# acdha/trivy

Hardware: AMD Instinct MI355X
Metric: secret-scan GB/s (builtin rules) at 1/2/4/8 MI355X; % of HBM peak (higher is better)
Workload: dtype u8

## Files before the change

include/trivy_secret.h:

```cpp
#ifndef TRIVY_SECRET_H
#define TRIVY_SECRET_H

#include <stddef.h>
#include <stdint.h>

#ifdef __cplusplus
extern "C" {
#endif

#define TSG_OK 0
#define TSG_ERR_CONFIG -1
#define TSG_ERR_ARG -2
#define TSG_ERR_GPU -3
#define TSG_ERR_NOMEM -4
#define TSG_ERR_INTERNAL -5

typedef struct tsg_allow_rule_desc {
  const char* id;
  const char* description;
  const char* regex;
  const char* path;
} tsg_allow_rule_desc;

typedef struct tsg_rule_desc {
// ... 230 lines not shown
int tsg_emulate_candidates(const tsg_ruleset* rs, const uint8_t* data, const uint64_t* offsets,
                           uint32_t nfiles, uint32_t chunk, uint32_t ext_cap, uint64_t items_cap,
                           uint32_t max_dense, uint32_t word_recs, uint32_t* records,
                           size_t records_cap, uint64_t* n_records);

int tsg_emulate_item_candidates(const tsg_ruleset* rs, const uint8_t* data, const uint64_t* offsets,
                                uint32_t nfiles, uint32_t chunk, uint32_t ext_cap, uint32_t* triples,
                                size_t triples_cap, uint64_t* n_triples);

int tsg_expand_candidates(const tsg_ruleset* rs, const uint8_t* data, const uint64_t* offsets,
                          uint32_t nfiles, const uint32_t* records, size_t n_records,
                          uint32_t* triples, size_t triples_cap, uint64_t* n_triples);

int tsg_layout_reference(const uint64_t* counts, uint32_t n_groups, uint64_t nchunks,
                         uint64_t items_cap, uint32_t max_dense, uint8_t* kind, uint64_t* totals);

int tsg_emulate_k1(const tsg_ruleset* rs, const uint8_t* data, const uint64_t* offsets,
                   uint32_t nfiles, uint32_t chunk, uint32_t* kw, size_t kw_len, uint32_t* ev,
                   size_t ev_len);

int tsg_emulate_k1f(const tsg_ruleset* rs, const uint8_t* data, const uint64_t* offsets,
                    uint32_t nfiles, uint32_t chunk, const uint32_t* quiet_ids, uint32_t nquiet,
                    uint32_t sample_kib, uint32_t* kw, size_t kw_len, uint32_t* ev, size_t ev_len,
                    uint64_t* stats);

int tsg_ruleset_rule_plan(const tsg_ruleset* rs, uint32_t rule, int32_t* group, int32_t* relax,
                          int64_t* max_len);

int tsg_ruleset_rule_anchor(const tsg_ruleset* rs, uint32_t rule, uint32_t* event, int64_t* evdist,
                            char* desc, size_t desc_len);

int tsg_ruleset_k1_literal(const tsg_ruleset* rs, uint32_t i, uint8_t* buf, uint32_t cap,
                           uint32_t* len, uint32_t* event);

int tsg_scan_batch_emulated(const tsg_ruleset* rs, const uint8_t* data, const uint64_t* offsets,
                            uint32_t nfiles, const char* paths, const uint64_t* path_offsets,
                            uint32_t chunk, tsg_result** out);

typedef struct tsg_layer tsg_layer;
typedef struct tsg_layer_view {
  const uint8_t* data;
  const uint64_t* offsets;
  uint32_t nfiles;
  const uint8_t* paths;
  const uint64_t* path_offsets;
  const char* opq;
  size_t opq_len;
  const char* wh;
  size_t wh_len;
  uint32_t walked;
} tsg_layer_view;
int tsg_layer_pack(const tsg_ruleset* rs, const uint8_t* tar, uint64_t tar_len,
                   const char* const* skip_files, uint32_t n_skip_files,
                   const char* const* skip_dirs, uint32_t n_skip_dirs, const char* config_path,
                   tsg_layer** out);
int tsg_layer_pack_shard(const tsg_ruleset* rs, const uint8_t* tar, uint64_t tar_len,
                         const char* const* skip_files, uint32_t n_skip_files,
                         const char* const* skip_dirs, uint32_t n_skip_dirs, const char* config_path,
                         uint32_t rank, uint32_t world, tsg_layer** out);
int tsg_layer_get(const tsg_layer* layer, tsg_layer_view* out);
typedef struct tsg_layer_range tsg_layer_range;
int tsg_layer_range_walk(const uint8_t* tar, uint64_t tar_len, uint32_t rank, uint32_t world,
                         tsg_layer_range** out, uint64_t info[4]);
int tsg_layer_range_sync(tsg_layer_range* range, uint64_t pos, uint64_t* end);
int tsg_layer_range_dirs(tsg_layer_range* range, const char* const* skip_dirs, uint32_t n_skip_dirs,
                         const char** out, uint64_t* out_len);
// ... 65 lines not shown
```

trivy_amd/_native.py:

```python
import ctypes as C
import os

LIB_PATH = os.path.join(os.path.dirname(os.path.abspath(__file__)), "libtrivy_secret.so")
if os.environ.get("TSG_LIB_VARIANT"):
    LIB_PATH = os.path.join(os.path.dirname(os.path.abspath(__file__)),
                            "libtrivy_secret_%s.so" % os.environ["TSG_LIB_VARIANT"])

TSG_OK = 0
TSG_ERR_CONFIG = -1
TSG_ERR_ARG = -2
TSG_ERR_GPU = -3
TSG_ERR_NOMEM = -4
TSG_ERR_INTERNAL = -5


class AllowRuleDesc(C.Structure):
    _fields_ = [("id", C.c_char_p), ("description", C.c_char_p), ("regex", C.c_char_p),
                ("path", C.c_char_p)]


class RuleDesc(C.Structure):
    _fields_ = [("id", C.c_char_p), ("category", C.c_char_p), ("title", C.c_char_p),
                ("severity", C.c_char_p), ("regex", C.c_char_p),
                ("keywords", C.POINTER(C.c_char_p)), ("n_keywords", C.c_uint32),
# ... 200 lines not shown
                                       C.POINTER(C.c_char_p), C.c_uint32, C.POINTER(C.c_char_p),
                                       C.c_uint32, C.c_char_p, C.POINTER(_P)]),
    ("tsg_layer_range_free", None, [_P]),
    ("tsg_fs_pack", C.c_int, [_P, C.c_char_p, C.POINTER(C.c_char_p), C.c_uint32,
                              C.POINTER(C.c_char_p), C.c_uint32, C.c_char_p, C.POINTER(_P)]),
    ("tsg_fs_pack_shard", C.c_int, [_P, C.c_char_p, C.POINTER(C.c_char_p), C.c_uint32,
                                    C.POINTER(C.c_char_p), C.c_uint32, C.c_char_p, C.c_uint32,
                                    C.c_uint32, C.POINTER(_P)]),
    ("tsg_layer_pack_slot", C.c_int, [_P, _P, C.c_uint64, C.POINTER(C.c_char_p), C.c_uint32,
                                      C.POINTER(C.c_char_p), C.c_uint32, C.c_char_p,
                                      C.POINTER(C.c_uint32), C.POINTER(_P)]),
    ("tsg_layer_range_pack_slot", C.c_int, [_P, _P, C.POINTER(C.c_char_p), C.c_uint32,
                                            C.POINTER(C.c_char_p), C.c_uint32,
                                            C.POINTER(C.c_char_p), C.c_uint32, C.c_char_p,
                                            C.POINTER(C.c_uint32), C.POINTER(_P)]),
    ("tsg_fs_pack_slot", C.c_int, [_P, C.c_char_p, C.POINTER(C.c_char_p), C.c_uint32,
                                   C.POINTER(C.c_char_p), C.c_uint32, C.c_char_p,
                                   C.POINTER(C.c_uint32), C.POINTER(_P)]),
    ("tsg_layer_scan", C.c_int, [_P, _P, C.c_uint64, C.POINTER(C.c_char_p), C.c_uint32,
                                 C.POINTER(C.c_char_p), C.c_uint32, C.c_char_p, C.POINTER(_P),
                                 C.POINTER(_P)]),
    ("tsg_fs_scan", C.c_int, [_P, C.c_char_p, C.POINTER(C.c_char_p), C.c_uint32,
                              C.POINTER(C.c_char_p), C.c_uint32, C.c_char_p, C.POINTER(_P),
                              C.POINTER(_P)]),
    ("tsg_layer_free", None, [_P]),
    ("tsg_go_sort_perm", C.c_int, [_P, _U64P, _I64P, C.c_uint32, C.POINTER(C.c_uint32)]),
    ("tsg_ruleset_rule_anchor", C.c_int, [_P, C.c_uint32, C.POINTER(C.c_uint32),
                                          C.POINTER(C.c_int64), C.c_char_p, C.c_size_t]),
    ("tsg_emulate_k1f", C.c_int, [_P, _P, _U64P, C.c_uint32, C.c_uint32, C.POINTER(C.c_uint32),
                                  C.c_uint32, C.c_uint32, C.POINTER(C.c_uint32), C.c_size_t,
                                  C.POINTER(C.c_uint32), C.c_size_t, C.POINTER(C.c_uint64)]),
    ("tsg_ruleset_k1_literal", C.c_int, [_P, C.c_uint32, C.c_char_p, C.c_uint32,
                                         C.POINTER(C.c_uint32), C.POINTER(C.c_uint32)]),
]

_lib = None


def lib():
    global _lib
    if _lib is None:
        if not os.path.exists(LIB_PATH):
            raise ImportError("libtrivy_secret.so is not built; run `python -m trivy_amd.build` "
                              "(expected at %s)" % LIB_PATH)
        L = C.CDLL(LIB_PATH)
        for name, res, args in SIGNATURES:
            fn = getattr(L, name)
            fn.restype = res
            fn.argtypes = args
        _lib = L
    return _lib


class NativeError(RuntimeError):
    def __init__(self, code, msg):
        super().__init__("%s (code %d)" % (msg, code))
        self.code = code


def knob(name, value=None):
    check(lib().tsg_test_knob(name.encode(), None if value is None else str(value).encode()))


def check(rc):
    if rc != TSG_OK:
        raise NativeError(rc, lib().tsg_last_error().decode("utf-8", "replace"))
# ... 2 lines not shown
```

trivy_amd/csrc/capi.cpp:

```cpp
#include <chrono>
#include <cstdio>
#include <cstdlib>
#include <cstring>
#include <exception>
#include <thread>

#include "internal.hpp"
#include "k1f.hpp"

namespace tsg {

static thread_local std::string g_last_error;

void set_error(const std::string& msg) { g_last_error = msg; }
int fail(int code, const std::string& msg) {
  g_last_error = msg;
  return code;
}

static void copy_err(const std::string& m, char* err, size_t len) {
  if (!err || len == 0) return;
  size_t n = std::min(len - 1, m.size());
  std::memcpy(err, m.data(), n);
  err[n] = 0;
// ... 402 lines not shown
      stats[0] = st[0];
      stats[1] = st[1];
      stats[2] = t.nlit;
      stats[3] = 0;
    }
    return TSG_OK;
  } catch (const std::bad_alloc&) {
    return fail(TSG_ERR_NOMEM, "out of memory");
  } catch (const std::exception& ex) {
    return fail(TSG_ERR_INTERNAL, ex.what());
  }
}

int tsg_ruleset_rule_plan(const tsg_ruleset* rs, uint32_t rule, int32_t* group, int32_t* relax,
                          int64_t* max_len) {
  if (!rs || rule >= rs->rs.rules.size()) return fail(TSG_ERR_ARG, "bad argument");
  const Plan& p = *rs->plan;
  if (group) *group = p.rule_hostonly[rule] ? -1 : p.rule_group[rule];
  if (relax) *relax = p.rule_relax[rule];
  if (max_len) *max_len = p.rule_maxlen[rule];
  return TSG_OK;
}

int tsg_ruleset_rule_anchor(const tsg_ruleset* rs, uint32_t rule, uint32_t* event, int64_t* evdist,
                            char* desc, size_t desc_len) {
  if (!rs || rule >= rs->rs.rules.size()) return fail(TSG_ERR_ARG, "bad argument");
  const Plan& p = *rs->plan;
  if (event) *event = p.rule_event[rule];
  if (evdist) *evdist = p.rule_evdist[rule];
  copy_err(p.rule_anchor[rule], desc, desc_len);
  return TSG_OK;
}

int tsg_ruleset_k1_literal(const tsg_ruleset* rs, uint32_t i, uint8_t* buf, uint32_t cap,
                           uint32_t* len, uint32_t* event) {
  if (!rs || (!buf && cap)) return fail(TSG_ERR_ARG, "bad argument");
  const Plan& p = *rs->plan;
  if (i >= p.k1_lits.size()) return fail(TSG_ERR_ARG, "no such K1 literal");
  const std::string& s = p.k1_lits[i];
  if (buf) std::memcpy(buf, s.data(), std::min<size_t>(cap, s.size()));
  if (len) *len = (uint32_t)s.size();
  if (event) *event = p.lit_event[i];
  return TSG_OK;
}

int tsg_go_sort_perm(const uint8_t* keys, const uint64_t* key_offsets, const int64_t* secondary,
                     uint32_t n, uint32_t* perm) {
  if ((n && (!keys || !key_offsets || !perm))) return fail(TSG_ERR_ARG, "bad argument");
  try {
    go_sort_perm(keys, key_offsets, secondary, n, perm);
    return TSG_OK;
  } catch (const std::bad_alloc&) {
    return fail(TSG_ERR_NOMEM, "out of memory");
  }
}

const uint8_t* tsg_result_data(const tsg_result* r, size_t* len) {
  if (!r) {
    if (len) *len = 0;
    return nullptr;
  }
  if (len) *len = r->buf.size();
  return (const uint8_t*)r->buf.data();
}

void tsg_result_free(tsg_result* r) { delete r; }
// ... 101 lines not shown
```

trivy_amd/csrc/k1f.cpp:

```cpp
#include "k1f.hpp"

#include <algorithm>
#include <cmath>
#include <cstring>
#include <memory>

namespace tsg {

namespace {

const uint32_t kBigram[] = {
#include "bigram.inc"
};

uint8_t fold(uint8_t c) { return (c >= 'A' && c <= 'Z') ? (uint8_t)(c + 32) : c; }

struct TextModel {
  std::vector<double> pi;
  std::vector<double> trans;
  TextModel() : pi(256, 0), trans(256 * 256, 0) {
    std::vector<double> cnt(256 * 256, 0.01);
    for (uint32_t e : kBigram) cnt[(e & 0xFF) * 256 + ((e >> 8) & 0xFF)] += std::exp2((double)(e >> 16) / 16.0) - 1.0;
    double tot = 0;
    for (int a = 0; a < 256; a++) {
// ... 299 lines not shown
          const uint32_t m = L.len - o >= 4 ? 0xFFFFFFFFu : (1u << (8 * (L.len - o))) - 1;
          ok = ((k1f_lower4(load4((int64_t)(s + o))) & m) == lv);
        }
        if (!ok) continue;
        stats[1]++;
        (*ev)[e / chunk] |= L.ev;
        if (L.kw >= 0) {
          const uint32_t f = (uint32_t)(std::upper_bound(bv.offsets, bv.offsets + F + 1, e) - bv.offsets) - 1;
          if (s >= bv.offsets[f]) (*kw)[(size_t)f * W + L.kw / 32] |= 1u << (L.kw % 32);
        }
      }
    }
  };
  uint32_t m1 = 0, m2 = 0;
  for (uint64_t P = 0; P < total; P += 16) {
    uint32_t r[16];
    for (int k = 0; k < 16; k++) r[k] = R((int64_t)(P + k));
    uint32_t any = 0;
    for (int g = 0; g < 4; g++) {
      const uint32_t gr = r[4 * g] | r[4 * g + 1] | r[4 * g + 2] | r[4 * g + 3];
      if (!(gr & 0xFFFFu)) continue;
      stats[0]++;
      any |= gr;
      for (int k = 4 * g; k < 4 * g + 4; k++)
        if (P + k < total && (r[k] & 0xFFFFu)) verify(P + k, r[k] & 0xFFFFu);
    }
    (void)any;
    const uint32_t m = k1f_flags(r[3], r[7], r[11], r[15]);
    const uint32_t rb = k1f_runs(m, m1, m2);
    if (rb) (*ev)[P / chunk] |= rb;
    m2 = m1;
    m1 = m;
  }
}

}
```

trivy_amd/csrc/kernels.hip:

```cpp
#include <hip/hip_runtime.h>

#include <algorithm>
#include <map>
#include <cstdlib>
#include <cstring>
#include <memory>
#include <vector>

#include "device.hpp"
#include "internal.hpp"
#include "k1f.hpp"

namespace tsg {

#define HIP_TRY(x)                                                                    \
  do {                                                                                \
    hipError_t e_ = (x);                                                              \
    if (e_ != hipSuccess)                                                             \
      return fail(TSG_ERR_GPU, std::string(#x) + ": " + hipGetErrorString(e_));       \
  } while (0)

constexpr int kStreams = 4;
constexpr int kK1Chains = 2;
constexpr int kK1Unroll = 8;
// ... 1445 lines not shown
    __syncthreads();
  }
}

struct GateArgs {
  const uint32_t* ev;
  uint64_t nchunks;
  uint32_t* evlist;
  uint32_t* nev;
  uint32_t ev_blocks;
  const uint32_t* kw;
  uint32_t F, W, GW;
  const unsigned long long* kwg;
  const unsigned long long* galw;
  unsigned long long* ggate;
  unsigned long long* clk;
  uint32_t kwg_lds;
};
constexpr uint32_t kKwgLdsMax = 48 * 1024;
__global__ void __launch_bounds__(kBlock) gates_kernel(GateArgs A) {
  extern __shared__ __attribute__((aligned(16))) uint8_t smem[];
  if (threadIdx.x == 0 && blockIdx.x < kStampBlocks)
    atomicMax(&A.clk[kClkGatesStart], ~(unsigned long long)wall_clock64());
  if (blockIdx.x < A.ev_blocks) {
    ev_compact_block(A.ev, A.nchunks, A.evlist, A.nev, blockIdx.x, A.ev_blocks);
  } else {
    const unsigned long long* kwg = A.kwg;
    if (A.kwg_lds) {
      stage16(smem, A.kwg, A.kwg_lds);
      __syncthreads();
      kwg = (const unsigned long long*)smem;
    }
    ggate_file((blockIdx.x - A.ev_blocks) * blockDim.x + threadIdx.x, A.kw, A.F, A.W, kwg, A.galw, A.GW, A.ggate);
  }
}

static inline size_t item_lds_host(uint32_t G, uint32_t GW) { return 256 * (size_t)GW + 8 * (size_t)G; }
constexpr uint32_t kItemKwgLdsMax = 16 * 1024;
struct ItemLds {
  const unsigned long long* gofbit;
  const uint32_t* gback;
  const uint32_t* gevents;
  const unsigned long long* kwg;
};
__device__ __forceinline__ uint32_t item_lds_bytes(const ItemArgs& A) { return 256 * A.GW + 8 * A.G + A.kwg_lds; }
__device__ __forceinline__ ItemLds item_lds_load(const ItemArgs& A, uint8_t* smem) {
  unsigned long long* gofbit = (unsigned long long*)smem;
  uint32_t* gback = (uint32_t*)(gofbit + 32 * A.GW);
  uint32_t* gevents = gback + A.G;
  for (uint32_t i = threadIdx.x; i < 32 * A.GW; i += blockDim.x) gofbit[i] = A.gofbit[i];
  for (uint32_t i = threadIdx.x; i < A.G; i += blockDim.x) {
    gback[i] = A.gback[i];
    gevents[i] = A.gevents[i];
  }
  const unsigned long long* kwg = A.kwg;
  if (A.kwg_lds) {
    unsigned long long* k = (unsigned long long*)(gevents + A.G);
    for (uint32_t i = threadIdx.x; i < A.kwg_lds / 8; i += blockDim.x) k[i] = A.kwg[i];
    kwg = k;
  }
  return ItemLds{gofbit, gback, gevents, kwg};
}

__device__ __forceinline__ unsigned long long file_gate(const ItemArgs& A, const ItemLds& T, uint32_t f, uint32_t w) {
  if (A.ggate) return A.ggate[(size_t)f * A.GW + w];
  const uint32_t* kwf = A.kw + (size_t)f * A.W;
// ... 1134 lines not shown
  int k2_grid = 0, k2_dense_grid = 0;
  bool k2_rich = false;
  hipEvent_t kernels_done = nullptr;
  bool kernels_done_valid = false;
  std::vector<void*> tables;
  DevK1 k1{};
  K1Host k1h;
  DevK1X k1x{};
  bool has_k1x = false;
  bool use_k1f = false;
  uint32_t k1f_maxlen = 4;
  DevK1F k1f{};
  K1FTables k1ft;
  DevBuf<uint32_t> d_fhits;
  DevBuf<uint32_t> d_hits;
  bool adapted = false;
  uint32_t hot_states = 0;
  uint32_t ev_hot = 0;
  uint64_t sample_bytes = 0;
  std::vector<uint32_t> lit_hits;
  std::vector<uint8_t> lit_quiet;
  std::shared_ptr<const std::vector<uint8_t>> kw_unknown;
  std::vector<uint32_t> h_galways, h_gevents;
  std::vector<unsigned long long> h_gofbit;
  std::vector<DevDFA> groups;
  DevDFA* d_groups = nullptr;
  uint32_t* d_gmask = nullptr;
  uint32_t* d_galways = nullptr;
  unsigned long long* d_kwg = nullptr;
  unsigned long long* d_galw = nullptr;
  uint32_t* d_gevents = nullptr;
  uint32_t* d_gback = nullptr;
  unsigned long long* d_gofbit = nullptr;
  std::vector<uint32_t> gback;
  uint32_t GW = 1, maxback = 0, max_lds = 0;
  ~DeviceRules() {
    (void)hipSetDevice(device);
    if (kernels_done) (void)hipEventDestroy(kernels_done);
    for (auto* p : tables) (void)hipFree(p);
  }
};

struct LaneState {
  DeviceRules* d = nullptr;
  hipStream_t st = nullptr;
  DevBuf<uint8_t> data_alloc;
  DevBuf<uint8_t> meta;
  const uint64_t* off = nullptr;
  DevBuf<uint32_t> cf;
  DevBuf<uint32_t> ev_bits;
  DevBuf<uint2> xlist;
  DevBuf<uint32_t> xcount;
  DevBuf<uint32_t> evlist;
  DevBuf<uint32_t> zclaim;
  DevBuf<unsigned long long> wtrace;
  size_t wtrace_n = 0;
  DevBuf<uint32_t> kw;
  DevBuf<unsigned long long> ggate;
  DevBuf<uint8_t> ovf;
  DevBuf<uint8_t> hascand;
  DevBuf<uint2> items;
  DevBuf<uint4> entries;
  DevBuf<uint4> dentries;
  DevBuf<DevCand> cand;
  DevBuf<uint32_t> counts;
  DevBuf<uint32_t> gcount;
// ... 291 lines not shown
    if ((rc = make_device_dfa(*gp.dfa, gp.rules, &dd, &r->tables))) return rc;
    r->max_lds = std::max(r->max_lds, dd.lds_bytes);
    r->groups.push_back(dd);
    gmask.insert(gmask.end(), gp.kwmask.begin(), gp.kwmask.end());
    galways.push_back(gp.always ? 1 : 0);
    gevents.push_back(gp.events);
    uint32_t back = group_back(gp, chunk);
    if (back > (uint32_t)kMaxBack) back = kMaxBack + 1;
    r->gback.push_back(back);
    if (back <= (uint32_t)kMaxBack) r->maxback = std::max(r->maxback, back);
    for (int b = 0; b < 32; b++)
      if (((gp.events >> b) & 1) || back > (uint32_t)kMaxBack) gofbit[b * r->GW + g / 64] |= 1ull << (g % 64);
  }
  r->max_lds = std::max<uint32_t>(r->max_lds, 16);
  {
    const size_t emit_lds = item_lds_host(G, r->GW) + kItemKwgLdsMax + 13 * (size_t)G + 16;
    if (emit_lds > 160 * 1024) return fail(TSG_ERR_INTERNAL, "too many rule groups for the item passes");
    if (emit_lds > 64 * 1024) {
      HIP_TRY(hipFuncSetAttribute((const void*)items_emit_kernel, hipFuncAttributeMaxDynamicSharedMemorySize, (int)emit_lds));
      HIP_TRY(hipFuncSetAttribute((const void*)items_count_kernel, hipFuncAttributeMaxDynamicSharedMemorySize, (int)emit_lds));
    }
  }
  if (r->max_lds > 64 * 1024) {
    HIP_TRY(hipFuncSetAttribute((const void*)k2_kernel, hipFuncAttributeMaxDynamicSharedMemorySize, (int)r->max_lds));
    HIP_TRY(hipFuncSetAttribute((const void*)k2_kernel_rich, hipFuncAttributeMaxDynamicSharedMemorySize, (int)r->max_lds));
    HIP_TRY(hipFuncSetAttribute((const void*)k2_dense_kernel, hipFuncAttributeMaxDynamicSharedMemorySize,
                                (int)r->max_lds));
  }
  if ((rc = upload_vec(gmask, &r->d_gmask, &r->tables))) return rc;
  if ((rc = upload_vec(galways, &r->d_galways, &r->tables))) return rc;
  if ((rc = upload_vec(gevents, &r->d_gevents, &r->tables))) return rc;
  if ((rc = upload_vec(r->gback, &r->d_gback, &r->tables))) return rc;
  if ((rc = upload_vec(gofbit, &r->d_gofbit, &r->tables))) return rc;
  {
    const uint32_t nkw = (uint32_t)p.kw_words * 32;
    std::vector<unsigned long long> kwg((size_t)nkw * r->GW, 0), galw(r->GW, 0);
    for (uint32_t g = 0; g < G; g++) {
      for (uint32_t k = 0; k < nkw; k++)
        if ((gmask[(size_t)g * p.kw_words + k / 32] >> (k % 32)) & 1) kwg[(size_t)k * r->GW + g / 64] |= 1ull << (g % 64);
      if (galways[g]) galw[g / 64] |= 1ull << (g % 64);
    }
    if ((rc = upload_vec(kwg, &r->d_kwg, &r->tables))) return rc;
    if ((rc = upload_vec(galw, &r->d_galw, &r->tables))) return rc;
  }
  r->h_galways = galways;
  r->h_gevents = gevents;
  r->h_gofbit = gofbit;
  if ((rc = upload_vec(r->groups, &r->d_groups, &r->tables))) return rc;
  hipDeviceProp_t prop;
  HIP_TRY(hipGetDeviceProperties(&prop, device));
  r->cus = prop.multiProcessorCount;
  r->grid = prop.multiProcessorCount * 8;
  HIP_TRY(hipEventCreateWithFlags(&r->kernels_done, hipEventDisableTiming | hipEventReleaseToDevice));
  int occ = 0;
  HIP_TRY(hipOccupancyMaxActiveBlocksPerMultiprocessor(&occ, (const void*)k2_kernel, kK2Block, r->max_lds));
  r->k2_grid = r->cus * std::max(occ, 1);
  {
    int occ_rich = 0;
    HIP_TRY(hipOccupancyMaxActiveBlocksPerMultiprocessor(&occ_rich, (const void*)k2_kernel_rich, kK2Block, r->max_lds));
    r->k2_rich = occ_rich >= 1 && occ_rich >= occ;
  }
  HIP_TRY(hipOccupancyMaxActiveBlocksPerMultiprocessor(&occ, (const void*)k2_dense_kernel, kBlock, r->max_lds));
  r->k2_dense_grid = r->cus * std::max(occ, 1);
  *out = r.release();
  return TSG_OK;
}
// ... 301 lines not shown
  IA.cf = l->cf;
  IA.ev = l->ev_bits;
  IA.ggate = l->ggate;
  IA.gofbit = r->d_gofbit;
  IA.gevents = r->d_gevents;
  IA.gback = r->d_gback;
  IA.nchunks = s.nchunks;
  IA.F = s.F;
  IA.G = s.G;
  IA.GW = r->GW;
  IA.chunk = s.C;
  IA.maxback = r->maxback;
  IA.count = l->gcount;
  IA.bcount = l->bcount;
  IA.cursor = l->cursor;
  IA.evlist = l->evlist;
  IA.nev = l->counts + kCntEvChunks;
  IA.evcap = (uint32_t)std::min<size_t>(l->evlist.cap, 0xFFFFFFFFu);
  IA.items = l->items;
  IA.kw = l->kw;
  IA.W = s.W;
  IA.kwg = r->d_kwg;
  IA.galw = r->d_galw;
  IA.clk = (unsigned long long*)(l->counts + kCntClk);
  if (s.work && k1f_list) {
    IA.ggate = nullptr;
  } else if (s.work) {
    const uint32_t cgrid = (uint32_t)std::min<uint64_t>((s.nchunks + kEvPer * kBlock - 1) / (kEvPer * kBlock), (uint64_t)r->grid);
    GateArgs GA{l->ev_bits, s.nchunks, l->evlist, l->counts + kCntEvChunks, cgrid, l->kw, s.F, s.W, r->GW, r->d_kwg, r->d_galw, l->ggate,
                (unsigned long long*)(l->counts + kCntClk), s.kwg_bytes <= kKwgLdsMax ? s.kwg_bytes : 0u};
    gates_kernel<<<cgrid + (s.F + kBlock - 1) / kBlock, kBlock, GA.kwg_lds, st>>>(GA);
    HIP_TRY(hipGetLastError());
  }
  if (s.work) {
    const int igrid = std::min(r->grid, r->cus * kItemsBpc);
    IA.kwg_lds = !IA.ggate && s.kwg_bytes <= kItemKwgLdsMax ? s.kwg_bytes : 0u;
    const size_t ilds = item_lds_host(s.G, r->GW) + IA.kwg_lds;
    hipLaunchKernelGGL(items_count_kernel, dim3(igrid), dim3(kBlock), ilds + s.G * sizeof(uint32_t) + 16, st, IA);
    HIP_TRY(hipGetLastError());
    LayoutArgs LA{l->gcount, s.G, s.nchunks, s.items_cap, s.max_dense, l->entries, l->counts + kCntListEntries,
                  l->dentries, l->counts + kCntDenseEntries, l->gskip, l->counts + kCntLayout};
    hipLaunchKernelGGL(items_emit_kernel, dim3(igrid), dim3(kBlock), ilds + 3 * s.G * sizeof(uint32_t) + s.G + 16, st, IA, LA);
    HIP_TRY(hipGetLastError());
  }
  HIP_TRY(hipEventRecord(out->ev[kEvK2], st));

  if (s.work) {
    K2Args A{};
    A.data = data;
    A.off = l->off;
    A.cf = l->cf;
    A.total = total;
    A.nchunks = s.nchunks;
    A.chunk = s.C;
    A.ext_cap = r->ext_cap;
    A.nfiles = s.F;
    A.kw = l->kw;
    A.kw_words = s.W;
    A.gmask = r->d_gmask;
    A.galways = r->d_galways;
    A.items = l->items;
    A.entries = l->entries;
    A.nentries = l->counts + kCntListEntries;
    A.dentries = l->dentries;
    A.ndentries = l->counts + kCntDenseEntries;
    A.cand = l->cand;
// ... 316 lines not shown
```

trivy_amd/csrc/plan.cpp:

```cpp
#include "plan.hpp"
#include "internal.hpp"
#include <deque>
#include <condition_variable>
#include <mutex>
#include <functional>

#include <algorithm>
#include <chrono>
#include <cstdio>
#include <cstdlib>
#include <atomic>
#include <map>
#include <unordered_map>
#include <unordered_set>
#include <set>
#include <thread>
#include <x86intrin.h>

namespace tsg {

static std::string ascii_lower(std::string s) {
  for (char& c : s)
    if (c >= 'A' && c <= 'Z') c = (char)(c + 32);
  return s;
// ... 42 lines not shown
    }
  }
}

static int x_pick(const std::string& l, int step, uint32_t* j0) {
  if (l.size() < (size_t)step + 3) return -1;
  const size_t last = std::min(l.size() - 3 - (size_t)step, (size_t)256 - (size_t)step);
  int best = -1;
  for (size_t j = 0; j <= last && best != 0; j++) {
    int c = 0;
    for (size_t t = j; t < j + (size_t)step; t++) c += common4().count(x_prefix4((const uint8_t*)l.data() + t)) ? 1 : 0;
    if (best < 0 || c < best) {
      best = c;
      *j0 = (uint32_t)j;
    }
  }
  return best;
}

namespace {

bool in_set(const uint64_t* set, const uint8_t* cls, int bit) {
  for (int c = 0; c < 128; c++)
    if (((set[c >> 6] >> (c & 63)) & 1) && !((cls[c] >> bit) & 1)) return false;
  return true;
}

struct Anchor {
  uint32_t kind = kEvAlways;
  std::string lit;
  int first_atom = 0;
  int64_t evdist = 0;
  std::string desc = "none";
};

Anchor choose_anchor(const Regexp& re, const Plan& p, bool literal_first) {
  const std::vector<AtomInfo> at = re.Atoms();
  const int n = (int)at.size();
  std::vector<int64_t> B(n + 1, 0);
  for (int i = 0; i < n; i++)
    B[i + 1] = (B[i] < 0 || at[i].max_bytes < 0) ? -1 : B[i] + at[i].max_bytes;
  Anchor best;
  auto take = [&](uint32_t kind, int t, int64_t len, const std::string& lit, const char* what) {
    Anchor a;
    a.kind = kind;
    a.lit = lit;
    if (B[t] >= 0) {
      a.first_atom = 0;
      a.evdist = B[t] + len - 1;
    } else {
      a.first_atom = t;
      a.evdist = len - 1;
    }
    a.desc = std::string(what) + (lit.empty() ? "" : " '" + lit + "'") + " at atom " +
             std::to_string(t) + (a.first_atom ? " (suffix)" : "");
    return a;
  };
  double best_score = 0;
  auto best_literal = [&]() {
    for (int i = 0; i < n;) {
      if (at[i].lit < 0) {
        i++;
        continue;
      }
      int j = i;
      std::string s;
      double score = 0;
      while (j < n && at[j].lit >= 0) {
        int c = at[j].lit;
        if (s.size() < 24) {
          s.push_back((char)c);
          score += (c >= 'a' && c <= 'z') ? 1.0 : (c >= '0' && c <= '9') ? 1.3 : 1.6;
        }
        j++;
      }
      if (score >= 3.0 && score > best_score) {
        best_score = score;
        best = take(1u << kEvLit0, i, (int64_t)s.size(), s, "literal");
      }
      i = j;
    }
  };
  if (literal_first) {
    best_literal();
    if (best_score >= 6.0) return best;
    best = Anchor();
    best_score = 0;
  }
  for (int bit = 0; bit < 2; bit++) {
    const int k = p.run_k[bit];
    for (int i = 0; i < n;) {
      if (!(at[i].ascii_only && in_set(at[i].set, p.run_cls, bit))) {
        i++;
        continue;
      }
      int j = i;
      int64_t run = 0;
      while (j < n && at[j].ascii_only && in_set(at[j].set, p.run_cls, bit)) run += at[j++].min_bytes;
      if (run >= k) return take(bit == 0 ? kEvRunU : kEvRunD, i, k, "", bit == 0 ? "run U" : "run D");
      i = j;
    }
  }
  best_literal();
  return best;
}

size_t product_states(const DFA& a, const DFA& b, size_t cap) {
  std::vector<uint8_t> seen((size_t)a.nstates * b.nstates, 0);
  std::vector<std::pair<uint32_t, uint32_t>> stack;
  uint16_t pcls[256][2];
  int np = 0;
  {
    std::map<std::pair<int, int>, int> idx;
    for (int c = 0; c < 256; c++) {
      auto k = std::make_pair((int)a.cls[c], (int)b.cls[c]);
      if (!idx.count(k)) idx[k] = np++;
      pcls[c][0] = (uint16_t)a.cls[c];
      pcls[c][1] = (uint16_t)b.cls[c];
    }
  }
  std::vector<int> rep;
  {
    std::set<std::pair<int, int>> done;
    for (int c = 0; c < 256; c++)
      if (done.insert({pcls[c][0], pcls[c][1]}).second) rep.push_back(c);
  }
  size_t n = 0;
  auto push = [&](uint32_t x, uint32_t y) {
    uint8_t& v = seen[(size_t)x * b.nstates + y];
    if (v) return;
    v = 1;
    n++;
// ... 173 lines not shown
        cur.push_back((uint32_t)r);
        cur_dfa = std::move(single[r]);
        continue;
      }
      std::vector<const Prog*> progs;
      for (uint32_t q : cur) progs.push_back(&p->rule_prog[q]);
      progs.push_back(&p->rule_prog[r]);
      std::string e;
      auto merged = build_dfa(progs, one, &e);
      if (getenv("TSG_PROF2"))
        fprintf(stderr, "merge %d+%d (nc %d,%d) -> %d %s\n", cur_dfa->nstates, single[r]->nstates,
                cur_dfa->nclasses, single[r]->nclasses, merged ? merged->nstates : -1,
                merged && fits(*merged, cur.size() + 1) ? "ok" : "FAIL");
      if (merged && fits(*merged, cur.size() + 1)) {
        cur.push_back((uint32_t)r);
        cur_dfa = std::move(merged);
      } else {
        flush();
        cur.push_back((uint32_t)r);
        cur_dfa = std::move(single[r]);
      }
    }
    flush();
  }

  if (tprof) {
    fprintf(stderr, "plan: grouping %.1f ms (%zu groups)\n", tms(tp), p->groups.size());
    for (size_t g = 0; g < p->groups.size(); g++)
      fprintf(stderr, "plan: group %zu: %zu rules, %d states x %d classes (%zu table bytes), events %#x\n", g,
              p->groups[g].rules.size(), p->groups[g].dfa->nstates, p->groups[g].dfa->nclasses,
              (size_t)p->groups[g].dfa->nstates * p->groups[g].dfa->nclasses * 2, p->groups[g].events);
  }
  tp = tnow();
  std::vector<char> litg(p->groups.size(), 0);
  for (size_t g = 0; g < p->groups.size(); g++) litg[g] = p->groups[g].events == (1u << kEvLit0);
  std::vector<char> kw_dropped(kws.size(), 0);
  std::vector<char> kw_hashed(kws.size(), 0), anchor_hashed(R, 0);
  auto build_k1 = [&](bool with_anchors) -> bool {
    std::vector<std::string> lits = kws;
    for (size_t k = 0; k < lits.size(); k++)
      if (kw_dropped[k] || kw_hashed[k]) lits[k] = never_literal();
    std::map<std::string, std::pair<int32_t, uint32_t>> xl;
    for (size_t k = 0; k < kws.size(); k++)
      if (kw_hashed[k]) xl[ascii_lower(kws[k])] = {(int32_t)k, 0u};
    std::vector<uint32_t> lit_event(lits.size(), 0);
    std::map<std::string, uint32_t> lid;
    for (size_t i = 0; i < lits.size(); i++) lid.emplace(lits[i], (uint32_t)i);
    int nlitgroups = 0;
    for (size_t gi = 0; gi < p->groups.size(); gi++) {
      GroupPlan& g = p->groups[gi];
      if (!litg[gi]) continue;
      if (!with_anchors) {
        g.events = kEvAlways;
        for (uint32_t r : g.rules) p->rule_event[r] = kEvAlways;
        continue;
      }
      const uint32_t bit = 1u << (kEvLit0 + (nlitgroups++ % kEvLitBits));
      g.events = bit;
      for (uint32_t r : g.rules) {
        p->rule_event[r] = bit;
        const std::string& s = anchor[r].lit;
        if (anchor_hashed[r]) {
          auto xi = xl.find(ascii_lower(s));
          if (xi == xl.end()) xl[ascii_lower(s)] = {-1, bit};
          else xi->second.second |= bit;
          continue;
        }
        auto it = lid.find(s);
        uint32_t id;
        if (it == lid.end()) {
          id = (uint32_t)lits.size();
          lid.emplace(s, id);
          lits.push_back(s);
          lit_event.push_back(0);
        } else {
          id = it->second;
        }
        lit_event[id] |= bit;
      }
    }
    DFAOptions o;
    o.max_states = 32767;
    o.with_noinject = false;
    std::string e;
    auto d = build_keyword_dfa(lits, o, &e);
    if (!d) return false;
    if ((size_t)d->nstates * d->nclasses * 2 > (size_t)opt.max_kw_table_bytes) return false;
    p->n_lit = (int)lits.size();
    p->lit_event = lit_event;
    p->k1_lits = lits;
// ... 825 lines not shown

void k1_reference(const Plan& plan, const BatchView& bv, uint32_t chunk, std::vector<uint32_t>* kw,
                  std::vector<uint32_t>* ev) {
  const uint32_t F = bv.nfiles;
  const uint64_t total = bv.offsets[F];
  const DFA& d = *plan.kw_dfa;
  const int nc = d.nclasses;
  const int W = plan.kw_words;
  kw->assign((size_t)F * W, 0);
  ev->assign((total + chunk - 1) / chunk, 0);
  uint32_t s = d.start[kCtxBOT];
  uint32_t cu = 0, cd = 0, f = 0;
  for (uint64_t p = 0; p < total; p++) {
    while (bv.offsets[f + 1] <= p) f++;
    const uint8_t c = bv.data[p];
    s = d.next[(size_t)s * nc + d.cls[c]];
    uint32_t e = 0;
    const uint32_t mi = d.eot_acc[s];
    if (mi) {
      const auto& m = d.masks[mi];
      const uint64_t avail = p - bv.offsets[f] + 1;
      for (int k = 0; k < plan.n_kw; k++)
        if (((m[k / 64] >> (k % 64)) & 1) && plan.kw_len[k] <= avail)
          (*kw)[(size_t)f * W + k / 32] |= 1u << (k % 32);
      e |= plan.kw_mask_events[mi];
    }
    cu = (plan.run_cls[c] & 1) ? cu + 1 : 0;
    cd = (plan.run_cls[c] & 2) ? cd + 1 : 0;
    if ((int)cu >= plan.run_k[0]) e |= kEvRunU;
    if ((int)cd >= plan.run_k[1]) e |= kEvRunD;
    (*ev)[p / chunk] |= e;
  }
  k1x_reference(plan, bv, chunk, kw, ev);
}

void k1x_reference(const Plan& plan, const BatchView& bv, uint32_t chunk, std::vector<uint32_t>* kw,
                   std::vector<uint32_t>* ev) {
  if (plan.x_lits.empty()) return;
  const uint64_t total = bv.offsets[bv.nfiles];
  std::unordered_map<uint32_t, std::vector<uint32_t>> by4;
  for (size_t i = 0; i < plan.x_lits.size(); i++) by4[x_prefix4((const uint8_t*)plan.x_lits[i].data())].push_back((uint32_t)i);
  auto low = [](uint8_t c) -> uint8_t { return (c >= 'A' && c <= 'Z') ? (uint8_t)(c + 32) : c; };
  for (uint64_t p = 0; p + 4 <= total; p++) {
    const uint8_t b4[4] = {low(bv.data[p]), low(bv.data[p + 1]), low(bv.data[p + 2]), low(bv.data[p + 3])};
    auto it = by4.find(x_prefix4(b4));
    if (it == by4.end()) continue;
    for (uint32_t i : it->second) {
      const std::string& L = plan.x_lits[i];
      if (p + L.size() > total) continue;
      size_t t = 4;
      while (t < L.size() && low(bv.data[p + t]) == (uint8_t)L[t]) t++;
      if (t < L.size()) continue;
      const uint64_t q = p + L.size() - 1;
      (*ev)[q / chunk] |= plan.x_event[i];
      if (plan.x_kw[i] >= 0) {
        const uint32_t f = (uint32_t)(std::upper_bound(bv.offsets, bv.offsets + bv.nfiles + 1, q) - bv.offsets) - 1;
        if (p >= bv.offsets[f]) (*kw)[(size_t)f * plan.kw_words + plan.x_kw[i] / 32] |= 1u << (plan.x_kw[i] % 32);
      }
    }
  }
}

static void emulate_records(const DFA& d, uint32_t gi, const std::vector<uint32_t>& rules, const uint8_t* data,
                            uint32_t f, uint64_t fs, uint64_t fe, uint64_t a, uint64_t b, uint32_t ext_cap,
                            bool body_words, bool tail_words, std::vector<Candidate>* out) {
  const uint32_t nc = (uint32_t)d.nclasses, ncd = std::max<uint32_t>(2, nc);
// ... 199 lines not shown
```

trivy_amd/csrc/plan.hpp:

```cpp
#pragma once
#include <cstdint>
#include <functional>
#include <memory>
#include <string>
#include <vector>

#include "dfa.hpp"
#include "scanner.hpp"

namespace tsg {

enum KwMode : uint8_t { kKwAlways = 0, kKwBits = 1, kKwUnknown = 2 };

constexpr uint32_t kEvRunU = 1u;
constexpr uint32_t kEvRunD = 2u;
constexpr int kEvLit0 = 2;
constexpr int kEvLitBits = 29;
constexpr uint32_t kEvAlways = 1u << 31;

struct GroupPlan {
  std::unique_ptr<DFA> dfa;
  std::vector<uint32_t> rules;
  std::vector<uint32_t> kwmask;
  bool always = false;
  uint32_t events = kEvAlways;
  int64_t evdist = 0;
};

struct Plan {
  std::unique_ptr<DFA> kw_dfa;
  int n_kw = 0;
  int n_lit = 0;
  int kw_words = 1;
  int fb_kw0 = 0;
  std::vector<uint32_t> kw_mask_events;
  std::vector<uint32_t> lit_event;
  std::vector<std::string> k1_lits;
  std::vector<uint16_t> kw_len;
  std::vector<std::string> x_lits;
  std::vector<int32_t> x_kw;
  std::vector<uint32_t> x_event;
  int x_step = 1;
  std::vector<uint8_t> x_j0;
  uint8_t run_cls[256] = {0};
  int run_k[2] = {32, 12};
  int warm = 32;
  std::vector<uint32_t> rule_event;
  std::vector<int64_t> rule_evdist;
  std::vector<int> rule_first_atom;
  std::vector<std::string> rule_anchor;
  std::vector<uint8_t> rule_kw_mode;
  std::vector<std::vector<uint32_t>> rule_kws;
  std::vector<GroupPlan> groups;
  std::vector<int> rule_group;
  std::vector<uint8_t> rule_hostonly;
  std::vector<int64_t> rule_maxlen;
  std::vector<int> rule_relax;
  std::vector<int> rule_atoms;
  std::vector<int64_t> rule_winback;
  std::vector<Prog> rule_prog;
  std::vector<std::unique_ptr<DFA>> rule_rev;
  std::vector<std::unique_ptr<DFA>> rule_fold_dfa;
  std::unique_ptr<DFA> fold_all_dfa;
  std::vector<uint32_t> fold_rules;
  std::unique_ptr<DFA> allow_path_dfa;
};

struct PlanOptions {
  int max_group_states = 1024;
  int max_group_table_bytes = 48 * 1024;
  int max_rules_per_group = 64;
  int max_kw_table_bytes = 96 * 1024;
  bool anchors = true;
};

std::unique_ptr<Plan> build_plan(const Ruleset& rs, const PlanOptions& opt, std::string* err);

constexpr uint32_t kCandWhole = 0xFFFFFFFFu;
// ... 74 lines not shown

void resolve_batch(const Ruleset& rs, const Plan& plan, const BatchView& b,
                   const KernelOutputView& ko, int nthreads, BatchResult* out);

void scan_batch_cpu(const Ruleset& rs, const BatchView& b, int nthreads,
                    std::vector<FileResult>* out);

struct EmuOptions {
  uint32_t max_back = 0xFFFFFFFFu;
  bool layout = false;
  uint64_t items_cap = 0;
  uint32_t max_dense = 0;
  uint64_t cand_cap = ~0ull;
};
struct EmuStats {
  uint64_t candidates = 0;
  LayoutTotals layout;
};
void emulate_kernels(const Plan& plan, const BatchView& b, uint32_t chunk, uint32_t ext_cap,
                     KernelOutput* ko, std::vector<uint64_t>* group_item_bytes = nullptr,
                     const EmuOptions* opt = nullptr, EmuStats* st = nullptr);

void emulate_candidates(const Plan& plan, const BatchView& b, uint32_t chunk, uint32_t ext_cap, uint64_t items_cap,
                        uint32_t max_dense, bool word_recs, std::vector<Candidate>* out);

void expand_candidate(const Plan& plan, const BatchView& b, const Candidate& c, std::vector<Candidate>* out);

void emulate_items(const Plan& plan, const BatchView& b, uint32_t chunk, const uint32_t* kw,
                   const std::vector<uint32_t>& ev, uint32_t max_back,
                   const std::function<void(uint32_t g, uint32_t f, uint64_t c)>& visit);

void k1_reference(const Plan& plan, const BatchView& b, uint32_t chunk,
                  std::vector<uint32_t>* kw, std::vector<uint32_t>* ev);
void k1x_reference(const Plan& plan, const BatchView& b, uint32_t chunk,
                   std::vector<uint32_t>* kw, std::vector<uint32_t>* ev);

inline uint32_t x_prefix4(const uint8_t* b) {
  return (uint32_t)b[0] | (uint32_t)b[1] << 8 | (uint32_t)b[2] << 16 | (uint32_t)b[3] << 24;
}
constexpr int kXDwordBits = 15;
constexpr uint32_t kXDwords = 1u << kXDwordBits;
constexpr uint32_t kXFold = 0x20202020u;
inline uint32_t x_fold(uint32_t w) { return w | kXFold; }
inline uint32_t x_hash(uint32_t w) { return w * 2654435761u; }
inline uint32_t x_dword(uint32_t h) { return h >> (32 - kXDwordBits); }
inline uint32_t x_bits(uint32_t h) { return 1u << ((h >> 12) & 31) | 1u << ((h >> 7) & 31); }

inline uint32_t group_back(const GroupPlan& g, uint32_t chunk) {
  return (uint32_t)((g.evdist + chunk - 1) / chunk);
}

}
```

trivy_amd/secret.py:

```python
import ctypes as C
import json
import os
import struct
from dataclasses import dataclass, field
from typing import List, Optional

import numpy as np
import yaml

from . import _native as N

_RULES_JSON = os.path.join(os.path.dirname(os.path.abspath(__file__)), "rules",
                           "builtin_rules.json")


class ConfigError(ValueError):
    """secrets config decode / regexp compile error (scanner.go:74-77, 286-288)."""


def _check_regex(src):
    h = C.c_void_p()
    err = C.create_string_buffer(512)
    rc = N.lib().tsg_regex_compile(src.encode("utf-8", "surrogateescape"), C.byref(h), err, 512)
    if rc != N.TSG_OK:
# ... 277 lines not shown
        u64p, u32p = C.POINTER(C.c_uint64), C.POINTER(C.c_uint32)
        args = (self.handle, C.c_void_p(batch.data.ctypes.data), batch.offsets.ctypes.data_as(u64p),
                batch.nfiles, chunk, int(ext_cap))
        n = C.c_uint64()
        N.check(N.lib().tsg_emulate_item_candidates(*args, None, 0, C.byref(n)))
        tri = np.zeros((max(n.value, 1), 3), dtype=np.uint32)
        N.check(N.lib().tsg_emulate_item_candidates(*args, tri.ctypes.data_as(u32p), n.value, None))
        return tri[:n.value]

    def expand_candidates(self, batch, records):
        rec = np.ascontiguousarray(records, dtype=np.uint32).reshape(-1, 3)
        u64p, u32p = C.POINTER(C.c_uint64), C.POINTER(C.c_uint32)
        args = (self.handle, C.c_void_p(batch.data.ctypes.data), batch.offsets.ctypes.data_as(u64p),
                batch.nfiles, rec.ctypes.data_as(u32p), len(rec))
        n = C.c_uint64()
        N.check(N.lib().tsg_expand_candidates(*args, None, 0, C.byref(n)))
        tri = np.zeros((max(n.value, 1), 3), dtype=np.uint32)
        N.check(N.lib().tsg_expand_candidates(*args, tri.ctypes.data_as(u32p), n.value, None))
        return tri[:n.value]

    def candidate_stats(self, batch, chunk):
        per_rule = np.zeros(max(len(self.Rules), 1), dtype=np.uint64)
        per_group = np.zeros(max(self.info()["n_groups"], 1), dtype=np.uint64)
        u64p = C.POINTER(C.c_uint64)
        N.check(N.lib().tsg_emulate_candidate_stats(
            self.handle, C.c_void_p(batch.data.ctypes.data), batch.offsets.ctypes.data_as(u64p),
            batch.nfiles, chunk, per_rule.ctypes.data_as(u64p), per_group.ctypes.data_as(u64p)))
        return per_rule[:len(self.Rules)], per_group[:self.info()["n_groups"]]

    def rule_group(self, rule):
        g, relax, ml = C.c_int32(), C.c_int32(), C.c_int64()
        N.check(N.lib().tsg_ruleset_rule_plan(self.handle, rule, C.byref(g), C.byref(relax), C.byref(ml)))
        return g.value

    def k1_literals(self):
        out = []
        buf = C.create_string_buffer(1 << 16)
        n, ev = C.c_uint32(), C.c_uint32()
        while N.lib().tsg_ruleset_k1_literal(self._h, len(out), buf, len(buf), C.byref(n), C.byref(ev)) == 0:
            out.append((buf.raw[:n.value], ev.value))
        return out

    def k1f_emulate(self, batch, chunk, quiet=(), sample_kib=0):
        import numpy as np
        W = (self.info()["n_keywords"] + 31) // 32
        kw = np.zeros(batch.nfiles * W, dtype=np.uint32)
        ev = np.zeros((int(batch.offsets[-1]) + chunk - 1) // chunk, dtype=np.uint32)
        q = np.array(list(quiet) or [0], dtype=np.uint32)
        st = np.zeros(4, dtype=np.uint64)
        u32p = C.POINTER(C.c_uint32)
        N.check(N.lib().tsg_emulate_k1f(self.handle, C.c_void_p(batch.data.ctypes.data),
                                        batch.offsets.ctypes.data_as(C.POINTER(C.c_uint64)),
                                        batch.nfiles, chunk, q.ctypes.data_as(u32p), len(quiet),
                                        sample_kib, kw.ctypes.data_as(u32p), kw.size, ev.ctypes.data_as(u32p),
                                        ev.size, st.ctypes.data_as(C.POINTER(C.c_uint64))))
        return kw.reshape(batch.nfiles, W), ev, {"groups": int(st[0]), "arrivals": int(st[1]),
                                                 "records": int(st[2])}

    def AllowPath(self, path):
        b = _b(path)
        rc = N.lib().tsg_ruleset_allow_path(self._h, b, len(b))
        if rc < 0:
            N.check(rc)
        return rc == 1

    def Scan(self, args):
# ... 538 lines not shown
```

Baseline: 56.74.

## Refine coarse run-U events into per-class run events with a GPU refine kernel

```diff
diff --git a/include/trivy_secret.h b/include/trivy_secret.h
--- a/include/trivy_secret.h
+++ b/include/trivy_secret.h
@@ -286,6 +286,8 @@
 
 int tsg_ruleset_k1_literal(const tsg_ruleset* rs, uint32_t i, uint8_t* buf, uint32_t cap,
                            uint32_t* len, uint32_t* event);
+
+int tsg_ruleset_run_classes(const tsg_ruleset* rs, uint32_t* n, uint8_t* cls, uint8_t* k);
 
 int tsg_scan_batch_emulated(const tsg_ruleset* rs, const uint8_t* data, const uint64_t* offsets,
                             uint32_t nfiles, const char* paths, const uint64_t* path_offsets,
diff --git a/trivy_amd/_native.py b/trivy_amd/_native.py
--- a/trivy_amd/_native.py
+++ b/trivy_amd/_native.py
@@ -256,6 +256,7 @@
                                   C.POINTER(C.c_uint32), C.c_size_t, C.POINTER(C.c_uint64)]),
     ("tsg_ruleset_k1_literal", C.c_int, [_P, C.c_uint32, C.c_char_p, C.c_uint32,
                                          C.POINTER(C.c_uint32), C.POINTER(C.c_uint32)]),
+    ("tsg_ruleset_run_classes", C.c_int, [_P, C.POINTER(C.c_uint32), _P, _P]),
 ]
 
 _lib = None
diff --git a/trivy_amd/csrc/capi.cpp b/trivy_amd/csrc/capi.cpp
--- a/trivy_amd/csrc/capi.cpp
+++ b/trivy_amd/csrc/capi.cpp
@@ -458,6 +458,18 @@
   return TSG_OK;
 }
 
+int tsg_ruleset_run_classes(const tsg_ruleset* rs, uint32_t* n, uint8_t* cls, uint8_t* k) {
+  if (!rs) return fail(TSG_ERR_ARG, "bad argument");
+  const Plan& p = *rs->plan;
+  if (n) *n = (uint32_t)p.n_refine;
+  if (cls) std::memcpy(cls, p.refine_cls, 256);
+  if (k) {
+    std::memset(k, 0, 8);
+    std::memcpy(k, p.refine_k, kMaxRefine);
+  }
+  return TSG_OK;
+}
+
 int tsg_ruleset_k1_literal(const tsg_ruleset* rs, uint32_t i, uint8_t* buf, uint32_t cap,
                            uint32_t* len, uint32_t* event) {
   if (!rs || (!buf && cap)) return fail(TSG_ERR_ARG, "bad argument");
diff --git a/trivy_amd/csrc/k1f.cpp b/trivy_amd/csrc/k1f.cpp
--- a/trivy_amd/csrc/k1f.cpp
+++ b/trivy_amd/csrc/k1f.cpp
@@ -355,6 +355,7 @@
     m2 = m1;
     m1 = m;
   }
-}
-
-}
+  refine_run_events(p, bv.data, total, chunk, ev);
+}
+
+}
diff --git a/trivy_amd/csrc/kernels.hip b/trivy_amd/csrc/kernels.hip
--- a/trivy_amd/csrc/kernels.hip
+++ b/trivy_amd/csrc/kernels.hip
@@ -1501,6 +1501,79 @@
       kwg = (const unsigned long long*)smem;
     }
     ggate_file((blockIdx.x - A.ev_blocks) * blockDim.x + threadIdx.x, A.kw, A.F, A.W, kwg, A.galw, A.GW, A.ggate);
+  }
+}
+
+constexpr uint32_t kRefineGroup = 64;
+static_assert(kRefineMaxK - 1 <= 2 * (int)kRefineGroup && 2 * kRefineGroup <= (uint32_t)kPad && kMaxRefine <= 4,
+              "the look-behind stays inside the pad; one counter byte per class");
+struct RefineArgs {
+  const uint8_t* data;
+  uint64_t total, nchunks;
+  uint32_t chunk;
+  uint32_t back;
+  uint32_t* ev;
+  const uint32_t* evlist;
+  const uint32_t* nev;
+  uint32_t evcap;
+  const uint32_t* tab;
+  uint32_t bias;
+};
+template <bool kHit>
+__device__ __forceinline__ void refine_word(const uint32_t* __restrict__ tab, const uint4 v, uint32_t nbytes,
+                                            uint32_t bias, uint32_t& cnt, uint32_t& hit) {
+  const uint32_t w[4] = {v.x, v.y, v.z, v.w};
+#pragma unroll
+  for (uint32_t i = 0; i < 16; i++) {
+    if (i < nbytes) {
+      const uint32_t m = tab[(w[i >> 2] >> (8 * (i & 3))) & 0xFFu];
+      cnt = ((cnt + 0x01010101u) & m) | (bias & ~m);
+      if (kHit) hit |= cnt;
+    }
+  }
+}
+__device__ __forceinline__ uint32_t refine_clamp(uint32_t cnt) {
+  const uint32_t top = cnt & 0x80808080u;
+  return cnt & ~((top >> 7) * 0x7Fu);
+}
+__global__ void __launch_bounds__(kBlock) refine_kernel(RefineArgs A) {
+  __shared__ uint32_t s_tab[256];
+  for (uint32_t i = threadIdx.x; i < 256; i += blockDim.x) s_tab[i] = A.tab[i];
+  __syncthreads();
+  const uint32_t nev = min(*A.nev, A.evcap);
+  for (uint32_t t = blockIdx.x * blockDim.x + threadIdx.x; t < nev; t += gridDim.x * blockDim.x) {
+    const uint32_t e = A.evlist[t];
+    if (e >= A.nchunks || !(A.ev[e] & kEvRunU)) continue;
+    const uint64_t a = (uint64_t)e * A.chunk, b = min(A.total, a + A.chunk);
+    const uint8_t* p = A.data + a;
+    const int64_t n = (int64_t)(b - a);
+    uint32_t cnt = A.bias, hit = 0;
+    int64_t q = -(int64_t)A.back;
+    uint4 v[4], nx[4];
+#pragma unroll
+    for (uint32_t i = 0; i < 4; i++) v[i] = nx[i] = *(const uint4*)(p + q + 16 * i);
+    for (; q + (int64_t)kRefineGroup <= n; q += kRefineGroup) {
+      if (q + 2 * (int64_t)kRefineGroup <= n) {
+#pragma unroll
+        for (uint32_t i = 0; i < 4; i++) nx[i] = *(const uint4*)(p + q + kRefineGroup + 16 * i);
+      }
+      if (q < 0) {
+#pragma unroll
+        for (uint32_t i = 0; i < 4; i++) refine_word<false>(s_tab, v[i], 16, A.bias, cnt, hit);
+      } else {
+#pragma unroll
+        for (uint32_t i = 0; i < 4; i++) refine_word<true>(s_tab, v[i], 16, A.bias, cnt, hit);
+      }
+      cnt = refine_clamp(cnt);
+#pragma unroll
+      for (uint32_t i = 0; i < 4; i++) v[i] = nx[i];
+    }
+    for (; q < n; q += 16)
+      refine_word<true>(s_tab, *(const uint4*)(p + q), (uint32_t)min((int64_t)16, n - q), A.bias, cnt, hit);
+    uint32_t bits = 0;
+#pragma unroll
+    for (int j = 0; j < kMaxRefine; j++) bits |= ((hit >> (8 * j + 7)) & 1) ? refine_bit(j) : 0u;
+    if (bits) atomicOr(&A.ev[e], bits);
   }
 }
 
@@ -2701,6 +2774,8 @@
   uint32_t* d_gevents = nullptr;
   uint32_t* d_gback = nullptr;
   unsigned long long* d_gofbit = nullptr;
+  uint32_t* d_refine = nullptr;
+  uint32_t refine_bias = 0, refine_back = 0;
   std::vector<uint32_t> gback;
   uint32_t GW = 1, maxback = 0, max_lds = 0;
   ~DeviceRules() {
@@ -3058,6 +3133,22 @@
   if ((rc = upload_vec(gevents, &r->d_gevents, &r->tables))) return rc;
   if ((rc = upload_vec(r->gback, &r->d_gback, &r->tables))) return rc;
   if ((rc = upload_vec(gofbit, &r->d_gofbit, &r->tables))) return rc;
+  if (p.n_refine) {
+    std::vector<uint32_t> tab(256, 0);
+    uint32_t maxk = 0;
+    if (p.n_refine > kMaxRefine) return fail(TSG_ERR_INTERNAL, "more refined run classes than counter bytes");
+    for (int j = 0; j < p.n_refine; j++) {
+      if (p.refine_k[j] < 1 || p.refine_k[j] > kRefineMaxK || (p.refine_cls[0] >> j & 1))
+        return fail(TSG_ERR_INTERNAL, "bad refined run class");
+      maxk = std::max<uint32_t>(maxk, p.refine_k[j]);
+      r->refine_bias |= (uint32_t)(128 - p.refine_k[j]) << (8 * j);
+      for (int b = 0; b < 256; b++)
+        if ((p.refine_cls[b] >> j) & 1) tab[b] |= 0xFFu << (8 * j);
+    }
+    r->refine_back = (maxk - 1 + kRefineGroup - 1) / kRefineGroup * kRefineGroup;
+    if (r->refine_back < kRefineGroup) r->refine_back = kRefineGroup;
+    if ((rc = upload_vec(tab, &r->d_refine, &r->tables))) return rc;
+  }
   {
     const uint32_t nkw = (uint32_t)p.kw_words * 32;
     std::vector<unsigned long long> kwg((size_t)nkw * r->GW, 0), galw(r->GW, 0);
@@ -3425,6 +3516,13 @@
     gates_kernel<<<cgrid + (s.F + kBlock - 1) / kBlock, kBlock, GA.kwg_lds, st>>>(GA);
     HIP_TRY(hipGetLastError());
   }
+  if (s.work && r->d_refine) {
+    RefineArgs RA{data, total, s.nchunks, s.C, r->refine_back, l->ev_bits, l->evlist, l->counts + kCntEvChunks,
+                  (uint32_t)std::min<size_t>(l->evlist.cap, 0xFFFFFFFFu), r->d_refine, r->refine_bias};
+    const int rgrid = (int)std::max<uint64_t>(1, std::min<uint64_t>((s.nchunks + kBlock - 1) / kBlock, (uint64_t)r->cus * 4));
+    refine_kernel<<<rgrid, kBlock, 0, st>>>(RA);
+    HIP_TRY(hipGetLastError());
+  }
   if (s.work) {
     const int igrid = std::min(r->grid, r->cus * kItemsBpc);
     IA.kwg_lds = !IA.ggate && s.kwg_bytes <= kItemKwgLdsMax ? s.kwg_bytes : 0u;
diff --git a/trivy_amd/csrc/plan.cpp b/trivy_amd/csrc/plan.cpp
--- a/trivy_amd/csrc/plan.cpp
+++ b/trivy_amd/csrc/plan.cpp
@@ -98,6 +98,8 @@
   int first_atom = 0;
   int64_t evdist = 0;
   std::string desc = "none";
+  uint64_t rset[2] = {0, 0};
+  int rk = 0;
 };
 
 Anchor choose_anchor(const Regexp& re, const Plan& p, bool literal_first) {
@@ -162,8 +164,24 @@
       }
       int j = i;
       int64_t run = 0;
-      while (j < n && at[j].ascii_only && in_set(at[j].set, p.run_cls, bit)) run += at[j++].min_bytes;
-      if (run >= k) return take(bit == 0 ? kEvRunU : kEvRunD, i, k, "", bit == 0 ? "run U" : "run D");
+      uint64_t set[2] = {0, 0};
+      while (j < n && at[j].ascii_only && in_set(at[j].set, p.run_cls, bit)) {
+        set[0] |= at[j].set[0];
+        set[1] |= at[j].set[1];
+        run += at[j++].min_bytes;
+      }
+      if (run >= k && bit == 0) {
+        bool whole = true;
+        for (int c = 0; c < 128; c++) whole &= !(p.run_cls[c] & 1) || ((set[c >> 6] >> (c & 63)) & 1);
+        if (whole) return take(kEvRunU, i, k, "", "run U");
+        const int rk = (int)std::min<int64_t>(run, kRefineMaxK);
+        Anchor a = take(kEvRunU, i, rk, "", "run U");
+        a.rset[0] = set[0];
+        a.rset[1] = set[1];
+        a.rk = rk;
+        return a;
+      }
+      if (run >= k) return take(kEvRunD, i, k, "", "run D");
       i = j;
     }
   }
@@ -403,6 +421,81 @@
               (size_t)p->groups[g].dfa->nstates * p->groups[g].dfa->nclasses * 2, p->groups[g].events);
   }
   tp = tnow();
+  {
+    struct Cls {
+      uint64_t s[2];
+      int k;
+      double w;
+    };
+    std::vector<Cls> cls;
+    std::vector<int> rule_cls(R, -1);
+    for (size_t r = 0; r < R; r++) {
+      if (p->rule_group[r] < 0 || p->rule_event[r] != kEvRunU || anchor[r].rk == 0) continue;
+      const Anchor& a = anchor[r];
+      size_t c = 0;
+      while (c < cls.size() && !(cls[c].s[0] == a.rset[0] && cls[c].s[1] == a.rset[1] && cls[c].k == a.rk)) c++;
+      if (c == cls.size()) cls.push_back({{a.rset[0], a.rset[1]}, a.rk, 0.0});
+      cls[c].w += 1;
+      rule_cls[r] = (int)c;
+    }
+    int nu = 0;
+    for (int c = 0; c < 128; c++) nu += p->run_cls[c] & 1;
+    auto rate = [&](const uint64_t* s, int k) {
+      const int n = __builtin_popcountll(s[0]) + __builtin_popcountll(s[1]);
+      return std::exp((double)k * std::log((double)n / nu));
+    };
+    std::vector<int> into(cls.size());
+    for (size_t c = 0; c < cls.size(); c++) into[c] = (int)c;
+    size_t live = cls.size();
+    while (live > (size_t)kMaxRefine) {
+      double best = 0;
+      int bi = -1, bj = -1;
+      for (size_t i = 0; i < cls.size(); i++) {
+        if (into[i] != (int)i) continue;
+        for (size_t j = i + 1; j < cls.size(); j++) {
+          if (into[j] != (int)j) continue;
+          const uint64_t m[2] = {cls[i].s[0] | cls[j].s[0], cls[i].s[1] | cls[j].s[1]};
+          const int k = std::min(cls[i].k, cls[j].k);
+          const double grow = rate(m, k) * (cls[i].w + cls[j].w) - rate(cls[i].s, cls[i].k) * cls[i].w -
+                              rate(cls[j].s, cls[j].k) * cls[j].w;
+          if (bi < 0 || grow < best) {
+            best = grow;
+            bi = (int)i;
+            bj = (int)j;
+          }
+        }
+      }
+      cls[bi].s[0] |= cls[bj].s[0];
+      cls[bi].s[1] |= cls[bj].s[1];
+      cls[bi].k = std::min(cls[bi].k, cls[bj].k);
+      cls[bi].w += cls[bj].w;
+      for (size_t c = 0; c < cls.size(); c++)
+        if (into[c] == bj) into[c] = bi;
+      live--;
+    }
+    std::vector<int> slot(cls.size(), -1);
+    for (size_t c = 0; c < cls.size(); c++) {
+      if (into[c] != (int)c) continue;
+      const int j = p->n_refine++;
+      slot[c] = j;
+      p->refine_k[j] = (uint8_t)cls[c].k;
+      for (int b = 0; b < 128; b++)
+        if ((cls[c].s[b >> 6] >> (b & 63)) & 1) p->refine_cls[b] |= (uint8_t)(1u << j);
+    }
+    for (size_t r = 0; r < R; r++) {
+      if (rule_cls[r] < 0) continue;
+      const int j = slot[into[rule_cls[r]]];
+      p->rule_event[r] = refine_bit(j);
+      p->rule_anchor[r] += " (class " + std::to_string(j) + ", k " + std::to_string(p->refine_k[j]) + ")";
+    }
+    if (p->n_refine)
+      for (auto& g : p->groups) {
+        if (g.events != kEvRunU) continue;
+        g.events = 0;
+        for (uint32_t r : g.rules) g.events |= p->rule_event[r];
+      }
+  }
+  const int lit_bits = kEvLitBits - p->n_refine;
   std::vector<char> litg(p->groups.size(), 0);
   for (size_t g = 0; g < p->groups.size(); g++) litg[g] = p->groups[g].events == (1u << kEvLit0);
   std::vector<char> kw_dropped(kws.size(), 0);
@@ -426,7 +519,7 @@
         for (uint32_t r : g.rules) p->rule_event[r] = kEvAlways;
         continue;
       }
-      const uint32_t bit = 1u << (kEvLit0 + (nlitgroups++ % kEvLitBits));
+      const uint32_t bit = 1u << (kEvLit0 + (nlitgroups++ % lit_bits));
       g.events = bit;
       for (uint32_t r : g.rules) {
         p->rule_event[r] = bit;
@@ -1318,6 +1411,25 @@
     (*ev)[p / chunk] |= e;
   }
   k1x_reference(plan, bv, chunk, kw, ev);
+  refine_run_events(plan, bv.data, total, chunk, ev);
+}
+
+void refine_run_events(const Plan& plan, const uint8_t* data, uint64_t total, uint32_t chunk,
+                       std::vector<uint32_t>* ev) {
+  if (!plan.n_refine) return;
+  for (uint64_t c = 0; c < ev->size(); c++) {
+    if (!((*ev)[c] & kEvRunU)) continue;
+    const uint64_t a = c * chunk, b = std::min<uint64_t>(total, a + chunk);
+    uint32_t cnt[kMaxRefine] = {0}, bits = 0;
+    for (uint64_t q = a > (uint64_t)(kRefineMaxK - 1) ? a - (kRefineMaxK - 1) : 0; q < b; q++) {
+      const uint8_t m = plan.refine_cls[data[q]];
+      for (int j = 0; j < plan.n_refine; j++) {
+        cnt[j] = ((m >> j) & 1) ? cnt[j] + 1 : 0;
+        if (q >= a && cnt[j] >= plan.refine_k[j]) bits |= refine_bit(j);
+      }
+    }
+    (*ev)[c] |= bits;
+  }
 }
 
 void k1x_reference(const Plan& plan, const BatchView& bv, uint32_t chunk, std::vector<uint32_t>* kw,
diff --git a/trivy_amd/csrc/plan.hpp b/trivy_amd/csrc/plan.hpp
--- a/trivy_amd/csrc/plan.hpp
+++ b/trivy_amd/csrc/plan.hpp
@@ -16,6 +16,9 @@
 constexpr uint32_t kEvRunD = 2u;
 constexpr int kEvLit0 = 2;
 constexpr int kEvLitBits = 29;
+constexpr int kMaxRefine = 4;
+constexpr int kRefineMaxK = 127;
+constexpr uint32_t refine_bit(int j) { return 1u << (kEvLit0 + kEvLitBits - 1 - j); }
 constexpr uint32_t kEvAlways = 1u << 31;
 
 struct GroupPlan {
@@ -44,6 +47,9 @@
   std::vector<uint8_t> x_j0;
   uint8_t run_cls[256] = {0};
   int run_k[2] = {32, 12};
+  int n_refine = 0;
+  uint8_t refine_cls[256] = {0};
+  uint8_t refine_k[kMaxRefine] = {0};
   int warm = 32;
   std::vector<uint32_t> rule_event;
   std::vector<int64_t> rule_evdist;
@@ -184,6 +190,8 @@
 
 void k1_reference(const Plan& plan, const BatchView& b, uint32_t chunk,
                   std::vector<uint32_t>* kw, std::vector<uint32_t>* ev);
+void refine_run_events(const Plan& plan, const uint8_t* data, uint64_t total, uint32_t chunk,
+                       std::vector<uint32_t>* ev);
 void k1x_reference(const Plan& plan, const BatchView& b, uint32_t chunk,
                    std::vector<uint32_t>* kw, std::vector<uint32_t>* ev);
 
diff --git a/trivy_amd/secret.py b/trivy_amd/secret.py
--- a/trivy_amd/secret.py
+++ b/trivy_amd/secret.py
@@ -333,6 +333,14 @@
         g, relax, ml = C.c_int32(), C.c_int32(), C.c_int64()
         N.check(N.lib().tsg_ruleset_rule_plan(self.handle, rule, C.byref(g), C.byref(relax), C.byref(ml)))
         return g.value
+
+    def run_classes(self):
+        n = C.c_uint32()
+        cls = np.zeros(256, dtype=np.uint8)
+        k = np.zeros(8, dtype=np.uint8)
+        N.check(N.lib().tsg_ruleset_run_classes(self.handle, C.byref(n), C.c_void_p(cls.ctypes.data),
+                                                C.c_void_p(k.ctypes.data)))
+        return cls, k[:n.value].astype(np.int64), [1 << (30 - j) for j in range(n.value)]
 
     def k1_literals(self):
         out = []
```

Result: no change. 56.56, median of 2 (-0.3%).
